# Matrixeigs/PowerSystemsReliabilityAssessment

Measured on AMD Instinct MI355X. Metric: Monte Carlo DC-OPF scenarios/sec (RTS-24 HL2 non-sequential), higher is better.
Workload: dtype f64

## Files before the change

powersystemsreliabilityassessment_amd/csrc/relmc_debug.hip:

```cpp
#include <cstdio>
#include <cstring>
#include <memory>

#include "relmc_ctx.h"
#include "relmc_shape_rts24.h"

using namespace relmc_host;

extern "C" {

int32_t relmc_debug_schedule(const relmc_ctx* ctx, int32_t* out9)
{
    if (!ctx || !out9 || !ctx->has_case) return RELMC_ERR_INVALID;
    auto fill = [&](const auto& C) {
        int ntask = 0;
        for (int p = 0; p < C.npass; ++p) ntask += C.pass_ntask[p];
        out9[0] = C.npass_upd; out9[1] = C.npass_inv; out9[2] = C.npass - C.npass_upd - C.npass_inv; out9[3] = C.noff;
        out9[4] = C.nzero; out9[5] = (int)C.nws; out9[6] = (int)ctx->lds_bytes; out9[7] = ctx->blocks_per_cu; out9[8] = ntask;
        if (verbose()) fprintf(stderr, "relmc: modelled LDS conflict cycles per Newton step %ld -> %ld\n", ctx->conflict_before, ctx->conflict_after);
        if (verbose()) fprintf(stderr, "relmc: longest line / injection list per bus slot: %d %d / %d %d\n", (int)C.maxdeg_s[0], (int)C.maxdeg_s[1], (int)C.maxinj_s[0], (int)C.maxinj_s[1]);
        if (verbose()) { fprintf(stderr, "relmc: tasks per pass:"); for (int p = 0; p < C.npass; ++p) fprintf(stderr, " %d", (int)C.pass_ntask[p]); fprintf(stderr, "\n"); }
    };
    if (ctx->tile == 0) fill(ctx->hcase24); else fill(ctx->hcase96);
    return RELMC_OK;
// ... 32 lines not shown
int32_t relmc_debug_phase_cycles(relmc_ctx* ctx, unsigned long long* out8)
{
    if (!ctx || !out8) return RELMC_ERR_INVALID;
    for (int k = 0; k < 8; ++k) out8[k] = 0;
    if (!ctx->dtiming.get() || ctx->timing_waves <= 0) return RELMC_OK;
    std::vector<unsigned long long> h((size_t)ctx->timing_waves * 8);
    HIP_TRY(ctx, hipMemcpy(h.data(), ctx->dtiming.get(), h.size() * sizeof(unsigned long long), hipMemcpyDeviceToHost));
    for (int w = 0; w < ctx->timing_waves; ++w) for (int k = 0; k < 8; ++k) out8[k] += h[(size_t)w * 8 + k];
    return RELMC_OK;
}

int32_t relmc_debug_norm_trips(relmc_ctx* ctx, unsigned long long* out2)
{
    if (!ctx || !out2) return RELMC_ERR_INVALID;
    out2[0] = out2[1] = 0;
    if (!ctx->dtiming.get() || ctx->timing_waves <= 0) return RELMC_OK;
    std::vector<unsigned long long> h((size_t)ctx->timing_waves * 2);
    HIP_TRY(ctx, hipMemcpy(h.data(), ctx->dtiming.get() + (size_t)ctx->timing_waves * 8, h.size() * sizeof(unsigned long long), hipMemcpyDeviceToHost));
    for (int w = 0; w < ctx->timing_waves; ++w) for (int k = 0; k < 2; ++k) out2[k] += h[(size_t)w * 2 + k];
    return RELMC_OK;
}

int32_t relmc_debug_trace(relmc_ctx* ctx, double* out, int32_t n_doubles)
{
    if (!ctx || !out || n_doubles < 0) return RELMC_ERR_INVALID;
    for (int k = 0; k < n_doubles; ++k) out[k] = 0.0;
    if (!ctx->dtiming.get() || n_doubles > 8 * 65536) return RELMC_OK;
    HIP_TRY(ctx, hipMemcpy(out, ctx->dtiming.get(), sizeof(double) * n_doubles, hipMemcpyDeviceToHost));
    return RELMC_OK;
}

int32_t relmc_debug_shape(const relmc_case_desc* d, const int32_t* order_hint, int32_t n_hint, int32_t* case_out, int32_t* static_out)
{
    if (static_out) ShapeRts24::values(static_out);
    if (case_out) {
        if (!d) return RELMC_ERR_INVALID;
        SymOpts so = sym_opts_default();
        if (order_hint && n_hint > 0) { so.order_hint = order_hint; so.n_hint = n_hint; }
        std::string err;
        SymGeom g;
        const int rc = with_symbolic(d, 0, so, g, err, [&](const auto& C) { shape_of(C, g.stash_off, g.scen_doubles, case_out); return (int)RELMC_OK; });
        if (rc) return rc < 0 ? rc : -rc;
    }
    return SF_COUNT;
}

int64_t relmc_debug_stretch_len(int64_t batch, int64_t done, double beta, double beta_limit, int64_t round, int32_t* final_out)
{
    if (batch <= 0 || batch > kStretchMaxBatch || done < 0 || round < 0) return RELMC_ERR_INVALID;
    const Stretch s = stretch_length(batch, done, beta, beta_limit, stretch_per(batch), round);
    if (final_out) *final_out = s.final ? 1 : 0;
    return s.len;
}

int32_t relmc_debug_shape_path(const relmc_ctx* ctx)
{
    if (!ctx || !ctx->has_case) return RELMC_ERR_INVALID;
    return ctx->shape_static && !ctx->sw.dynamic_shape ? 1 : 0;
}

int32_t relmc_debug_tail_plan(int64_t n, int32_t waves, int64_t* a_begin, int64_t* a_end, int32_t* owner, int64_t* group)
{
    if (n < 0 || waves <= 0) return RELMC_ERR_INVALID;
    const TailPlan plan(n, waves);
    for (int64_t w = 0; w < waves; ++w) { if (a_begin) a_begin[w] = plan.begin(w); if (a_end) a_end[w] = plan.cut(w); }
    for (int64_t p = 0; p < plan.items(); ++p) { if (owner) owner[p] = (int32_t)plan.owner(p); if (group) group[p] = plan.group(p); }
    return plan.T;
}

int32_t relmc_debug_tail_groups(const relmc_ctx* ctx, int64_t* launches_out, int32_t* waves_out)
{
    if (!ctx) return RELMC_ERR_INVALID;
    if (launches_out) *launches_out = ctx->tail_launches;
    if (waves_out) *waves_out = ctx->has_case && ctx->tile == 0 ? ctx->num_cu * ctx->blocks_per_cu * Tile24::WPB : 0;
    return ctx->last_tail_groups;
}

// ... 17 lines not shown
```

powersystemsreliabilityassessment_amd/csrc/relmc_dev.h:

```cpp
#pragma once
#include <stdint.h>

namespace relmc {

template <int RW_, int BS_, int LS_, int IS_, int NCOMPMAX_, int MAXPASS_, int MAXOFF_, int WPB_>
struct TileT {
    static constexpr int RW = RW_;
    static constexpr int BS = BS_;
    static constexpr int LS = LS_;
    static constexpr int IS = IS_;
    static constexpr int NBT = BS_ * RW_;
    static constexpr int NLT = LS_ * RW_;
    static constexpr int NIT = IS_ * RW_;
    static constexpr int SPW = 64 / RW_;
    static constexpr int NCOMPMAX = NCOMPMAX_;
    static constexpr int OW = NCOMPMAX_ / 32;
    static constexpr int MAXPASS = MAXPASS_;
    static constexpr int MAXOFF = MAXOFF_;
    static constexpr int WPB = WPB_;
    static_assert(BS_ <= 2 && LS_ <= 3 && IS_ <= 4, "the per-lane flag word has room for 2 bus, 3 line and 4 injection slots");
};
using Tile24 = TileT<16, 2, 3, 4, 128, 96, 160, 4>;
using Tile96 = TileT<64, 2, 2, 3, 256, 64, 320, 8>;
constexpr int DEGMAX = 8;
// ... 10 lines not shown
    static constexpr int NBT = TL::NBT, NLT = TL::NLT, NIT = TL::NIT, NCOMPMAX = TL::NCOMPMAX, MAXPASS = TL::MAXPASS, MAXOFF = TL::MAXOFF, ROWL = TL::RW;
    int32_t nb, ng, nl, nd, ninj, ncomp, ref_bus, noff;
    double base_mva, total_load;
    uint32_t exist_mask;
    uint32_t nws;
    uint16_t off_rhs, off_p;
    uint16_t npass, npass_upd, npass_inv, nzero;
    uint16_t maxdeg, maxinj, base_connected, npass_updq;
    uint16_t maxdeg_s[2], maxinj_s[2];
    uint16_t npass_updh, pad3[3];
    uint64_t bwd_half;
    uint64_t b_line8[NBT];
    uint64_t b_inj8[NBT];
    double b_bsum[NBT];
    double l_b[NLT];
    double l_rate[NLT];
    uint32_t l_info[NLT];
    int32_t l_partner[NLT];
    uint16_t l_blk[NLT];
    alignas(16) double i_tab[NIT][4];
    uint32_t i_info[NIT];
    uint8_t b_nline[NBT];
    uint8_t b_line[NBT][DEGMAX];
    uint8_t b_ninj[NBT];
    uint8_t b_inj[NBT][BINJMAX];
    int16_t b_vinj[NBT];
    uint8_t b_ext[NBT];
    uint8_t b_lane[NBT];
    uint8_t b_int[NBT];
    uint32_t thr[NCOMPMAX];
    uint16_t zero_off[MAXOFF];
    uint8_t pass_ntask[MAXPASS];
    uint16_t task[MAXPASS][ROWL][4];
};

template <class TL>
struct PartialT {
    double dns, dns2;
    double shed[TL::IS];
    uint32_t n, nfail, nsing, ninf, nnc, iters;
    uint32_t cf_inj[TL::IS];
    uint32_t cf_line[TL::LS];
    uint32_t pad;
};

template <class TL>
struct TailRecT {
    double shed[64][TL::IS];
    double dns[TL::SPW];
    uint32_t flag[TL::SPW];
};

struct FailRec {
    unsigned long long unit;
    uint32_t weight, pad;
    uint32_t mask[8];
};

struct EvalArgs {
    uint64_t seed, first_index;
    int64_t n;
    int32_t policy, max_it;
    double feastol, gradtol, comptol, costtol, xi, sigma, z0, alpha_min, max_stepsize;
    const uint8_t* states;
    double* dns;
    double* nodal;
// ... 139 lines not shown
```

powersystemsreliabilityassessment_amd/csrc/relmc_kernels.hip:

```cpp
#include "relmc_devfn.h"
#include "relmc_shape_rts24.h"

namespace relmc {


constexpr int kPrioBit = 12;
constexpr int kMinWaves = 2;
#define DINF __builtin_inf()
#define RELOAD_FENCE() __asm__ volatile("" ::: "memory")
#define SLOT_FENCE() __builtin_amdgcn_sched_barrier(0)
#ifdef RELMC_PASS_NOUNROLL
#define PASS_LOOP _Pragma("nounroll")
#else
#define PASS_LOOP
#endif
constexpr int kPfMask = 0xc0;
constexpr int kPfMaskWide = 0xc6;
#define PFSITE(k) (((PF_MASK >> (k)) & 1) != 0)
constexpr int kShadowMask = 0xff;
constexpr int kShadowMaskWide = 0xff;
constexpr int kNormSplitMask = 0xff;
constexpr int kNormSplitMaskWide = 0;
#ifdef RELMC_ZERO_EXPLICIT
constexpr bool kZeroBySlot = false;
#else
constexpr bool kZeroBySlot = true;
#endif
#define PASS_IDLE(d) (((d).x & 0xffffu) == ((d).y >> 16))
#define PASS_IDLE_INV(d) ((d).y != 0u)
#ifdef RELMC_PHASE_TIMING
#define PT_DECL unsigned long long pt_[8] = {0, 0, 0, 0, 0, 0, 0, 0}, ptn_[2] = {0, 0}; unsigned long long pt0_ = __builtin_readcyclecounter();
#define PT_MARK(k) { const unsigned long long n_ = __builtin_readcyclecounter(); pt_[k] += n_ - pt0_; pt0_ = n_; }
#define PT_TRIP(k) ptn_[k] += 1;
#define PT_FLUSH if (a.timing && lane == 0) { for (int k = 0; k < 8; ++k) a.timing[((size_t)blockIdx.x * WPB + (tid >> 6)) * 8 + k] = pt_[k]; \
                                              for (int k = 0; k < 2; ++k) a.timing[(size_t)gridDim.x * WPB * 8 + ((size_t)blockIdx.x * WPB + (tid >> 6)) * 2 + k] = ptn_[k]; }
#else
#define PT_DECL
#define PT_MARK(k)
#define PT_TRIP(k)
#define PT_FLUSH
#endif
#if defined(RELMC_PHASE_TIMING) && defined(RELMC_PT_INIT)
#undef PT_MARK
#define PT_MARK(k) { const unsigned long long n_ = __builtin_readcyclecounter(); pt_[(k) == 7 ? 7 : 6] += n_ - pt0_; pt0_ = n_; }
#define PT_IMARK(k) { const unsigned long long n_ = __builtin_readcyclecounter(); pt_[k] += n_ - pt0_; pt0_ = n_; }
#else
#define PT_IMARK(k)
#endif

template <int MODE_, class TL, class SH = ShapeDynamic>
__global__ void __launch_bounds__(64 * TL::WPB, kMinWaves) relmc_eval_kernel(const DevCaseT<TL>* __restrict__ gcase, const EvalArgs a)
{
    constexpr int MODE = MODE_ == 5 ? 0 : (MODE_ == 6 ? 4 : MODE_);
    constexpr bool DENSE = MODE_ == 6;
    constexpr int PAIR_MASK = TL::RW == 16 ? kRpairMask : kRpairMaskWide;
#define PAIRSITE(k) (((PAIR_MASK >> (k)) & 1) != 0)
    constexpr int PF_MASK = TL::RW == 16 ? kPfMask : kPfMaskWide;
    constexpr bool SHADOW = (((TL::RW == 16 ? kShadowMask : kShadowMaskWide) >> MODE) & 1) != 0;
    constexpr bool NSPLIT = (((TL::RW == 16 ? kNormSplitMask : kNormSplitMaskWide) >> MODE) & 1) != 0;
    constexpr bool LSHARE = (((TL::RW == 16 ? kLineRcpShareMask : kLineRcpShareMaskWide) >> MODE) & 1) != 0 && PAIRSITE(0) && PAIRSITE(2) && PAIRSITE(6);
    constexpr bool ZSLOT = kZeroBySlot && (SH::kMask & SH::grp_nl) != 0 && (SH::kMask & SH::grp_ninj) != 0;
    constexpr int RW = TL::RW, BS = TL::BS, LS = TL::LS, IS = TL::IS, NBT = TL::NBT, WPB = TL::WPB, SPW = TL::SPW, OW = TL::OW;
    using DevCase = DevCaseT<TL>;
    using Partial = PartialT<TL>;
    extern __shared__ __attribute__((aligned(16))) unsigned char smem[];
    constexpr uint32_t OPT_BYTES = 128;
    double* const OPT = reinterpret_cast<double*>(smem);
#define A_(k, name) OPT[k]
    DevCase& C = *reinterpret_cast<DevCase*>(smem + OPT_BYTES);
    const DevCase& TASKSRC = *gcase;
    const DevCase& TABL = C;
    const DevCase& TABI = (RW == 64) ? *gcase : C;
    const DevCase& TABG = (RW == 64) ? *gcase : C;
    const int tid = threadIdx.x, lane = tid & 63, rlane = lane & (RW - 1), row = tid / RW;
    const uint32_t case_bytes = a.case_bytes;
    {
        const uint32_t* src = reinterpret_cast<const uint32_t*>(gcase);
        uint32_t* dst = reinterpret_cast<uint32_t*>(smem + OPT_BYTES);
        if (tid == 0) { OPT[0] = a.feastol; OPT[1] = a.gradtol; OPT[2] = a.comptol; OPT[3] = a.costtol; OPT[4] = a.xi; OPT[5] = a.sigma;
                        OPT[6] = a.z0; OPT[7] = a.alpha_min; OPT[8] = a.max_stepsize; OPT[9] = a.fail_threshold; }
        for (uint32_t i = tid; i < case_bytes / 4; i += 64 * WPB) dst[i] = src[i];
    }
    __syncthreads();
    double* const W = reinterpret_cast<double*>(smem + OPT_BYTES + ((case_bytes + 15u) & ~15u)) + (size_t)row * SHAPE(scen_doubles, a.scen_doubles);
    const int nlp = SHAPE(nl, C.nl), nip = SHAPE(ninj, C.ninj);
    double* const LR = W;
    double* const IR = W + 4 * (nlp + 1);
    const int maxdeg0 = SHAPE(maxdeg0, C.maxdeg_s[0]), maxdeg1 = SHAPE(maxdeg1, C.maxdeg_s[1]), maxinj0 = SHAPE(maxinj0, C.maxinj_s[0]), maxinj1 = SHAPE(maxinj1, C.maxinj_s[1]);
    double* const Stash = W + SHAPE(stash_off, a.stash_off) + 2 * rlane;
    const double* const StashJ = W + SHAPE(stash_off, a.stash_off);
    double* const Lam = W + SHAPE(stash_off, a.stash_off) + 2 * IS * RW + 2;
    uint32_t* const OB = reinterpret_cast<uint32_t*>(Lam + NBT);

    const int ng = SHAPE(ng, C.ng), ncomp = C.ncomp, nb = SHAPE(nb, C.nb);
    const bool bwd_all_half = SHAPE(bwd_all_half, __builtin_amdgcn_readfirstlane((uint32_t)(C.bwd_half != 0 ? 1u : 0u)) != 0);
    const int off_rhs = SHAPE(off_rhs, C.off_rhs), npu = SHAPE(npass_upd, C.npass_upd), npi = SHAPE(npass_inv, C.npass_inv), npass = SHAPE(npass, C.npass), nzero = SHAPE(nzero, C.nzero), npuh = SHAPE(npass_upd, C.npass_upd) - SHAPE(npass_updq, C.npass_updq), npuf = npuh - SHAPE(npass_updh, C.npass_updh);
    const double base = C.base_mva;
    const double eps = 2.220446049250313e-16;

    uint32_t linfo[LS]; int lpart[LS];
#pragma unroll
    for (int s = 0; s < LS; ++s) { const int l = RW * s + rlane; linfo[s] = C.l_info[l]; lpart[s] = C.l_partner[l]; }
    constexpr bool LTAB_LDS = (MODE == 1 || MODE == 2 || MODE == 4);
    constexpr bool ITAB_REG = RW == 64;
    double lbv_[LS], lrv_[LS], ihi_[IS], ilo_[IS];
#pragma unroll
    for (int s = 0; s < LS; ++s) { lbv_[s] = LTAB_LDS ? 0.0 : TABL.l_b[RW * s + rlane]; lrv_[s] = LTAB_LDS ? 0.0 : TABL.l_rate[RW * s + rlane]; }
#pragma unroll
    for (int s = 0; s < IS; ++s) { ihi_[s] = ITAB_REG ? TABI.i_tab[RW * s + rlane][0] : 0.0; ilo_[s] = ITAB_REG ? TABI.i_tab[RW * s + rlane][1] : 0.0; }
#define lb(s) (LTAB_LDS ? TABL.l_b[RW * (s) + rlane] : lbv_[s])
#define lr(s) (LTAB_LDS ? TABL.l_rate[RW * (s) + rlane] : lrv_[s])
#define IHL(s, j) (ITAB_REG ? d2{ihi_[s], ilo_[s]} : ld2(TABI.i_tab[j]))
#define ICOST(s, j) TABI.i_tab[j][2]
#define PLIST(t, bi) TABG.b_line8[bi]
#define JLIST(t, bi) TABG.b_inj8[bi]
    uint32_t iinfo[IS];
#pragma unroll
    for (int s = 0; s < IS; ++s) iinfo[s] = C.i_info[RW * s + rlane];
    int vb[BS];
#pragma unroll
    for (int t = 0; t < BS; ++t) vb[t] = C.b_lane[RW * t + rlane];

    Partial& PA = reinterpret_cast<Partial*>(a.partial)[(size_t)blockIdx.x * (64 * WPB) + tid];
    {
        PA.dns = 0.0; PA.dns2 = 0.0;
#pragma unroll
        for (int s = 0; s < IS; ++s) { PA.shed[s] = 0.0; PA.cf_inj[s] = 0; }
#pragma unroll
        for (int s = 0; s < LS; ++s) PA.cf_line[s] = 0;
        PA.n = 0; PA.nfail = 0; PA.nsing = 0; PA.ninf = 0; PA.nnc = 0; PA.iters = 0; PA.pad = 0;
    }
    uint32_t acc_n = 0, acc_it = 0;

    PT_DECL
    const int64_t ngroups = (a.n + SPW - 1) / SPW;
    const int64_t gwave = (int64_t)blockIdx.x * WPB + (tid >> 6);
    const int64_t gstride = (int64_t)gridDim.x * WPB;
    const bool prio_first = a.prio_mode == 1 ? blockIdx.x < (gridDim.x >> 1) : (a.prio_mode == 2 ? ((tid >> 8) & 1) == 0 : false);
    if (a.prio_mode != 0 && !prio_first) __builtin_amdgcn_s_setprio(1);
    constexpr bool WINDOWED = (MODE == 0 && RW == 16);
    uint32_t* const WIN = reinterpret_cast<uint32_t*>(smem + OPT_BYTES + ((case_bytes + 15u) & ~15u)) +
                          (size_t)SPW * WPB * SHAPE(scen_doubles, a.scen_doubles) * 2 + (size_t)(tid >> 6) * 256;
    uint8_t* const WINL = reinterpret_cast<uint8_t*>(smem + OPT_BYTES + ((case_bytes + 15u) & ~15u)) +
                          ((size_t)SPW * WPB * SHAPE(scen_doubles, a.scen_doubles) * 2 + (size_t)WPB * 256) * 4 + (size_t)(tid >> 6) * 64;
    int64_t wb_begin = gwave, wb_end = ngroups, wb_step = gstride;
    if (WINDOWED) {
        wb_begin = ngroups * gwave / gstride; wb_end = ngroups * (gwave + 1) / gstride; wb_step = 16;
    }
    static_assert(!WINDOWED || 80 + 4 * WPB <= OPT_BYTES, "one word per wavefront behind the ten option doubles");
    int* const TP = reinterpret_cast<int*>(smem + 80) + (tid >> 6);
    if (WINDOWED) { *TP = -1; RELOAD_FENCE(); }
    for (int64_t wb = wb_begin; WINDOWED || wb < wb_end; wb += wb_step) {
    int win_groups = 1, wg0 = 0;
    uint32_t win_valid = 0;
// ... 510 lines not shown
                        const double hp = pv - hl.x, hm = ILOV(s, hl.y) - pv;
                        const double lxp = ICOST(s, j) - Lam[iinfo[s] & 0xff] + (imup[s] - imum[s]);
                        if constexpr ((RW == 16 && kInjNform) || (RW == 64 && kInjNformWide)) {
                            const double N = __builtin_fma(imup[s], izm[s], imum[s] * izp[s]);
                            const double rN = frcp(N), zz = izp[s] * izm[s];
                            invD = zz * rN;
                            npd = __builtin_fma(lxp, zz, (imup[s] * hp + gamma) * izm[s] - (imum[s] * hm + gamma) * izp[s]) * rN;
                        } else {
                        double rzp, rzm; frcp_pair<PAIRSITE(1)>(izp[s], izm[s], rzp, rzm);
                        const double D = imup[s] * rzp + imum[s] * rzm;
                        const double np = lxp + (imup[s] * hp + gamma) * rzp - (imum[s] * hm + gamma) * rzm;
                        invD = frcp(D); npd = np * invD;
                        }
                        if constexpr (NORMS) {
                            mx_lx = vmax(mx_lx, __builtin_fabs(lxp));
                            mx_gh = vmax(mx_gh, vmax(hp, hm));
                            mx_z = vmax(mx_z, vmax(izp[s], izm[s]));
                            mx_lammu = vmax(mx_lammu, vmax(imup[s], imum[s]));
                        }
                    }
                    if (ZSLOT ? j <= nip : j < nip) IR[j] = pv;
                    st2(Stash + 2 * RW * s, invD, npd);
                    SLOT_FENCE();
                }
                PT_MARK(1)
                if (rlane == 0) {
                    if (!ZSLOT || nlp >= LS * RW) { st2(LR + 4 * nlp, 0.0, 0.0); st2(LR + 4 * nlp + 2, 0.0, 0.0); }
                    if (!ZSLOT || nip >= IS * RW) IR[nip] = 0.0;
                }
                uint32_t lblk_pf[LS]; uint32_t zo_pf = 0;
                if constexpr (PFSITE(1)) {
#pragma unroll
                    for (int s = 0; s < LS; ++s) lblk_pf[s] = C.l_blk[RW * s + rlane];
                    zo_pf = C.zero_off[rlane];
                }
                unsigned long long pl_pf[BS], pj_pf[BS];
                if constexpr (PFSITE(2)) {
#pragma unroll
                    for (int t = 0; t < BS; ++t) { const int bq = vb[t] < nb ? vb[t] : 0; pl_pf[t] = PLIST(t, bq); pj_pf[t] = JLIST(t, bq); }
                }
                double vown[LS];
                {
                    double gp[LS];
#pragma unroll
                    for (int s = 0; s < LS; ++s) gp[s] = LR[4 * (lpart[s] >= 0 ? lpart[s] : nlp)];
#pragma unroll
                    for (int s = 0; s < LS; ++s) vown[s] = (((linfo[s] >> 24) & LF_OWNER) && !L_PIN(s)) ? -(gown[s] + gp[s]) : 0.0;
                }
                double d00[BS], d11[BS], r0[BS], r1[BS];
#pragma unroll
                for (int t = 0; t < BS; ++t) {
                    const int bi = vb[t];
                    d00[t] = 0; d11[t] = 0; r0[t] = 0; r1[t] = 0;
                    if (bi < nb) {
                        double md = 0.0, lx = 0.0, nq_ = 0.0, bal = 0.0, E = 0.0, ssum = 0.0;
                        const unsigned long long pl = PFSITE(2) ? pl_pf[t] : PLIST(t, bi), pj = PFSITE(2) ? pj_pf[t] : JLIST(t, bi);
#pragma unroll
                        for (int e = 0; e < DEGMAX; e += 2) {
                            if (e >= (t == 0 ? maxdeg0 : maxdeg1)) break;
                            const uint32_t ent0 = (uint32_t)(pl >> (8 * e)) & 0xffu, ent1 = (uint32_t)(pl >> (8 * e + 8)) & 0xffu;
                            const int l0 = (int)(ent0 & 0x7f), l1 = (int)(ent1 & 0x7f);
                            const double sg0 = (ent0 & 0x80) ? -1.0 : 1.0, sg1 = (ent1 & 0x80) ? -1.0 : 1.0;
                            const d2 ra0 = ld2(LR + 4 * l0), rb0 = ld2(LR + 4 * l0 + 2), ra1 = ld2(LR + 4 * l1), rb1 = ld2(LR + 4 * l1 + 2);
                            md += ra0.x;
                            lx = __builtin_fma(sg0, ra0.y, lx);
                            nq_ = __builtin_fma(sg0, rb0.x, nq_);
                            bal = __builtin_fma(sg0, rb0.y, bal);
// ... 32 lines not shown
                }
                double o_ct = 0.0, o_cc = 0.0, o_am = 0.0;
                if constexpr (NSPLIT && PFSITE(7)) o_am = A_(7, alpha_min);
                RELOAD_FENCE();
                if constexpr (DENSE) {
                    const int n = 2 * nb, n1 = n + 1;
                    volatile double* A = a.dense + ((size_t)blockIdx.x * (WPB * SPW) + (size_t)(tid / RW)) * (size_t)a.dense_stride;
                    for (int e = rlane; e < n * n1; e += RW) A[e] = 0.0;
                    __threadfence_block();
#pragma unroll
                    for (int s = 0; s < LS; ++s) {
                        if ((linfo[s] >> 24) & LF_OWNER) {
                            const int f = linfo[s] & 0xff, t = (linfo[s] >> 8) & 0xff;
                            const int hi = f < t ? t : f, lo = f < t ? f : t;
                            const double c1 = L_C1Z(s) ? 0.0 : cBv[s], c2 = L_C2Z(s) ? 0.0 : cBv[s];
                            A[(2 * hi) * n1 + 2 * lo] = vown[s]; A[(2 * lo) * n1 + 2 * hi] = vown[s];
                            A[(2 * hi) * n1 + 2 * lo + 1] = c1; A[(2 * lo + 1) * n1 + 2 * hi] = c1;
                            A[(2 * hi + 1) * n1 + 2 * lo] = c2; A[(2 * lo) * n1 + 2 * hi + 1] = c2;
                        }
                    }
#pragma unroll
                    for (int t = 0; t < BS; ++t) {
                        const int bi = vb[t];
                        if (bi < nb) {
                            A[(2 * bi) * n1 + 2 * bi] = d00[t]; A[(2 * bi) * n1 + 2 * bi + 1] = cBd[t];
                            A[(2 * bi + 1) * n1 + 2 * bi] = cBd[t]; A[(2 * bi + 1) * n1 + 2 * bi + 1] = d11[t];
                            A[(2 * bi) * n1 + n] = r0[t]; A[(2 * bi + 1) * n1 + n] = r1[t];
                        }
                    }
                    __threadfence_block();
                } else {
#pragma unroll
                for (int s = 0; s < LS; ++s) {
                    if ((linfo[s] >> 24) & LF_OWNER) {
                        const double c1 = L_C1Z(s) ? 0.0 : cBv[s];
                        const double c2 = L_C2Z(s) ? 0.0 : cBv[s];
                        double* blk = W + (PFSITE(1) ? lblk_pf[s] : (uint32_t)C.l_blk[RW * s + rlane]);
                        st2(blk, vown[s], c1); st2(blk + 2, c2, 0.0);
                    }
                }
                if constexpr (PFSITE(1)) {
                    for (int z = rlane; z < nzero; z += RW) {
                        const uint32_t zn = C.zero_off[z + RW < TL::MAXOFF ? z + RW : z];
                        double* blk = W + zo_pf; st2(blk, 0.0, 0.0); st2(blk + 2, 0.0, 0.0);
                        zo_pf = zn;
                    }
                } else
                for (int z = rlane; z < nzero; z += RW) { double* blk = W + C.zero_off[z]; st2(blk, 0.0, 0.0); st2(blk + 2, 0.0, 0.0); }
#pragma unroll
                for (int t = 0; t < BS; ++t) {
                    const int bi = vb[t];
                    if (bi < nb) {
                        st2(W + 4 * bi, d00[t], cBd[t]); st2(W + 4 * bi + 2, cBd[t], d11[t]);
                        st2(W + off_rhs + 2 * bi, r0[t], r1[t]);
                    }
                }
                }

                PT_MARK(2)
                bool conv = false, xnan = false;
                if constexpr (NSPLIT) {
                    mx_x = x_inf; xnan = x_nan;
                    conv = NORMS && stage1;
                } else {
                    if constexpr (PFSITE(7)) { o_ct = A_(2, comptol); o_cc = A_(3, costtol); o_am = A_(7, alpha_min); }
                    mx_x = row_max<RW>(mx_x);
                    xnan = row_any<RW>(nanx, lane);
                    if constexpr (!PFSITE(7)) { o_ct = A_(2, comptol); o_cc = A_(3, costtol); }
                    conv = it > 0 && zmu < o_ct * (1.0 + mx_x) && __builtin_fabs(fval - f0) < o_cc * (1.0 + __builtin_fabs(f0));
                }
#ifdef RELMC_TRACE
                {
                    const double t_gh = row_max<RW>(mx_gh), t_z = row_max<RW>(mx_z), t_lx = row_max<RW>(mx_lx), t_lm = row_max<RW>(mx_lammu);
                    if (a.timing && blockIdx.x == 0 && tid == 0 && it < 60) {
                        double* o = reinterpret_cast<double*>(a.timing) + 8 * it;
                        o[0] = t_gh / (1.0 + vmax(mx_x, t_z)); o[1] = t_lx / (1.0 + t_lm); o[2] = zmu / (1.0 + mx_x);
                        o[3] = __builtin_fabs(fval - f0) / (1.0 + __builtin_fabs(f0)); o[4] = alphap; o[5] = alphad; o[6] = gamma; o[7] = fval;
                    }
                }
#endif
                if constexpr (NORMS) if (__any(conv)) {
                    mx_gh = row_max<RW>(mx_gh); mx_z = row_max<RW>(mx_z); mx_lx = row_max<RW>(mx_lx); mx_lammu = row_max<RW>(mx_lammu);
                    conv = conv && mx_gh < A_(0, feastol) * (1.0 + vmax(mx_x, mx_z)) && mx_lx < A_(1, gradtol) * (1.0 + mx_lammu);
                }
// ... 559 lines not shown
```

powersystemsreliabilityassessment_amd/csrc/relmc_schedule.hip:

```cpp
#include <algorithm>
#include <chrono>
#include <cmath>
#include <cstddef>
#include <cstdio>
#include <cstdlib>
#include <cstring>

#include "relmc_ctx.h"
#ifdef RELMC_DEV_SWITCHES
#include "relmc_dev_switches.h"
#endif

namespace relmc_host {

bool verbose()
{
    static const bool v = std::getenv("RELMC_VERBOSE") != nullptr;
    return v;
}

SymOpts sym_opts_default()
{
    SymOpts so;
#ifdef RELMC_DEV_SWITCHES
// ... 562 lines not shown
        }
        C.maxdeg = (uint16_t)maxdeg; C.maxinj = (uint16_t)maxinj;
        return RELMC_OK;
    }
    void bus_lanes()
    {
        for (int q = 0; q < NBT; ++q) C.b_lane[q] = 0xff;
        std::vector<int> slot_of(nb, 0);
        const int n1 = nb > ROWL ? nb - ROWL : 0;
        if (n1 > 0 && TL::BS == 2 && !so.no_bus_map) {
            int best_a = DEGMAX, best_b = BINJMAX, best_steps = 1 << 30;
            for (int a2 = 0; a2 <= DEGMAX; ++a2) for (int b2 = 0; b2 <= BINJMAX; ++b2) {
                int cnt = 0;
                for (int i = 0; i < nb; ++i) if (C.b_nline[i] <= a2 && C.b_ninj[i] <= b2) cnt++;
                const int steps = (a2 + 1) / 2 + (b2 + 1) / 2;
                if (cnt >= n1 && steps < best_steps) { best_steps = steps; best_a = a2; best_b = b2; }
            }
            std::vector<int> cand;
            for (int i = 0; i < nb; ++i) if (C.b_nline[i] <= best_a && C.b_ninj[i] <= best_b) cand.push_back(i);
            std::stable_sort(cand.begin(), cand.end(), [&](int x, int y) { return C.b_nline[x] + C.b_ninj[x] < C.b_nline[y] + C.b_ninj[y]; });
            for (int k = 0; k < n1; ++k) slot_of[cand[k]] = 1;
        } else {
            for (int i = 0; i < nb; ++i) slot_of[i] = i / ROWL;
        }
        int fill[TL::BS] = {};
        for (int i = 0; i < nb; ++i) {
            const int t = slot_of[i];
            C.b_lane[ROWL * t + fill[t]++] = (uint8_t)i;
            if (C.b_nline[i] > C.maxdeg_s[t]) C.maxdeg_s[t] = C.b_nline[i];
            if (C.b_ninj[i] > C.maxinj_s[t]) C.maxinj_s[t] = C.b_ninj[i];
        }
    }

    void base_connectivity()
    {
        std::vector<int> lab(nb); for (int i = 0; i < nb; ++i) lab[i] = i;
        auto find = [&](int x) { while (lab[x] != x) { lab[x] = lab[lab[x]]; x = lab[x]; } return x; };
        for (int l = 0; l < nl; ++l) { const int a2 = find(d->br_from[l]), b2 = find(d->br_to[l]); if (a2 != b2) lab[a2] = b2; }
        int roots = 0; for (int i = 0; i < nb; ++i) if (find(i) == i) roots++;
        C.base_connected = roots == 1 ? 1 : 0;
    }

    void thresholds()
    {
        for (int k = 0; k < ncomp; ++k) {
            double t = std::floor(d->unavail[k] * 4294967296.0);
            if (!(t > 0)) t = 0;
            if (t > 4294967295.0) t = 4294967295.0;
            C.thr[k] = d->always_up[k] ? 0u : (uint32_t)t;
        }
    }
    int geometry()
    {
        const uint32_t case_bytes = (uint32_t)offsetof(DevCaseT<TL>, task);
        const uint32_t lds_bytes = 128u + ((case_bytes + 15u) & ~15u) + (uint32_t)SPW * WPB * stride * (uint32_t)sizeof(double) + (ROWL == 16 ? (1024u + 64u) * WPB : 0u);
        if (lds_bytes > 160u * 1024u) return failx(RELMC_ERR_UNSUPPORTED, "relmc_case_load: case needs more than 160 KiB of LDS per workgroup");
        geom.stash_off = stash_off; geom.scen_doubles = stride; geom.lds_bytes = lds_bytes;
        return RELMC_OK;
    }
};

}

template <class TL>
int case_symbolic(const relmc_case_desc* d, DevCaseT<TL>& C, int order_variant, const SymOpts& so, SymGeom& geom, std::string& err)
{
    using S = Symbolic<TL>;
    using clock = std::chrono::steady_clock;
    auto ms = [](clock::time_point a, clock::time_point b) { return std::chrono::duration<double, std::milli>(b - a).count(); };
    S s(d, C, order_variant, so, geom, err);
    auto run = [&](std::initializer_list<int (S::*)()> steps) { for (auto step : steps) if (const int rc = (s.*step)()) return rc; return (int)RELMC_OK; };
    if (const int rc = run({&S::header, &S::elimination_order, &S::block_layout, &S::task_list})) return rc;
    const auto t_sched0 = clock::now();
    s.dependencies();
    if (const int rc = s.schedule()) return rc;
    const auto t_place0 = clock::now();
    if (verbose()) fprintf(stderr, "relmc: scheduling %.1f ms\n", ms(t_sched0, t_place0));
    s.place();
    if (verbose()) fprintf(stderr, "relmc: placement search %.1f ms\n", ms(t_place0, clock::now()));
    s.pass_forms();
    s.byte_offsets();
    if (const int rc = run({&S::shadow_idle_lanes, &S::pass_counts, &S::lines, &S::injections})) return rc;
    s.bus_lanes();
    s.base_connectivity();
    s.thresholds();
    return s.geometry();
}

template int case_symbolic<Tile24>(const relmc_case_desc*, DevCaseT<Tile24>&, int, const SymOpts&, SymGeom&, std::string&);
template int case_symbolic<Tile96>(const relmc_case_desc*, DevCaseT<Tile96>&, int, const SymOpts&, SymGeom&, std::string&);

constexpr long kPassWeight = 4;
template <class TL>
long schedule_cost(const DevCaseT<TL>& C, int32_t* lds_out, int32_t* passes_out)
{
    const int nbwd = (int)C.npass - (int)C.npass_upd - (int)C.npass_inv;
    const int nfull = (int)C.npass_upd - (int)C.npass_updh - (int)C.npass_updq;
    long lds = 10L * nfull + 7L * C.npass_updh + 6L * C.npass_updq + 6L * C.npass_inv;
    for (int k = 0; k < nbwd; ++k) lds += (k < 64 && ((C.bwd_half >> k) & 1ull)) ? 6 : 7;
    if (lds_out) *lds_out = (int32_t)lds;
    if (passes_out) *passes_out = (int32_t)C.npass;
    return lds + kPassWeight * (long)C.npass;
}
template <class TL>
int tune_order_impl(const relmc_case_desc* d, DevCaseT<TL>& C, int32_t evaluations, uint64_t seed, const int32_t* start, int32_t* order_out, int32_t* stats)
{
    const int nb = d->nb;
    SymOpts so = sym_opts_default();
    so.place_moves = 0;
    std::string err;
    SymGeom g;
    std::vector<int32_t> cur(nb), best(nb), cand(nb);
    int32_t lds = 0, np = 0;
    if (start) cur.assign(start, start + nb);
    else {
        const int rc = case_symbolic<TL>(d, C, 0, so, g, err);
// ... 105 lines not shown
```

powersystemsreliabilityassessment_amd/csrc/relmc_shape.h:

```cpp
#pragma once
#include <stdint.h>

#include "relmc_dev.h"

namespace relmc {

enum ShapeField {
    SF_RW = 0, SF_NB, SF_NG, SF_NL, SF_NINJ, SF_NZERO, SF_OFF_RHS, SF_NPASS_UPD, SF_NPASS_UPDH, SF_NPASS_UPDQ, SF_NPASS_INV, SF_NPASS,
    SF_MAXDEG0, SF_MAXDEG1, SF_MAXINJ0, SF_MAXINJ1, SF_BWD_ALL_HALF, SF_STASH_OFF, SF_SCEN_DOUBLES, SF_COUNT
};

enum ShapeGroup { SG_PASS = 1, SG_GATHER = 2, SG_DIM = 4, SG_OFF = 8, SG_ALL = 15 };
#define SHAPE(field, dyn) ((SH::kMask & SH::grp_##field) != 0 ? (decltype(+(dyn)))SH::field : (dyn))
struct ShapeGroups {
    static constexpr int grp_npass_upd = SG_PASS, grp_npass_updh = SG_PASS, grp_npass_updq = SG_PASS, grp_npass_inv = SG_PASS, grp_npass = SG_PASS, grp_bwd_all_half = SG_PASS,
                         grp_maxdeg0 = SG_GATHER, grp_maxdeg1 = SG_GATHER, grp_maxinj0 = SG_GATHER, grp_maxinj1 = SG_GATHER,
                         grp_nb = SG_DIM, grp_ng = SG_DIM, grp_nl = SG_DIM, grp_ninj = SG_DIM, grp_nzero = SG_DIM,
                         grp_off_rhs = SG_OFF, grp_stash_off = SG_OFF, grp_scen_doubles = SG_OFF;
};
struct ShapeDynamic : ShapeGroups {
    static constexpr int kMask = 0;
    static constexpr int nb = 0, ng = 0, nl = 0, ninj = 0, nzero = 0, off_rhs = 0, npass_upd = 0, npass_updh = 0, npass_updq = 0, npass_inv = 0, npass = 0,
                         maxdeg0 = 0, maxdeg1 = 0, maxinj0 = 0, maxinj1 = 0, bwd_all_half = 0, stash_off = 0, scen_doubles = 0;
};

template <class V, int MASK = SG_ALL>
struct ShapeStaticT : ShapeGroups {
    static constexpr int kMask = MASK;
    static constexpr int nb = V::nb, ng = V::ng, nl = V::nl, ninj = V::ninj, nzero = V::nzero, off_rhs = V::off_rhs, npass_upd = V::npass_upd, npass_updh = V::npass_updh,
                         npass_updq = V::npass_updq, npass_inv = V::npass_inv, npass = V::npass, maxdeg0 = V::maxdeg0, maxdeg1 = V::maxdeg1, maxinj0 = V::maxinj0,
                         maxinj1 = V::maxinj1, bwd_all_half = V::bwd_all_half, stash_off = V::stash_off, scen_doubles = V::scen_doubles;
    static void values(int32_t* out)
    {
        out[SF_RW] = V::rw; out[SF_NB] = V::nb; out[SF_NG] = V::ng; out[SF_NL] = V::nl; out[SF_NINJ] = V::ninj; out[SF_NZERO] = V::nzero;
        out[SF_OFF_RHS] = V::off_rhs; out[SF_NPASS_UPD] = V::npass_upd; out[SF_NPASS_UPDH] = V::npass_updh; out[SF_NPASS_UPDQ] = V::npass_updq;
        out[SF_NPASS_INV] = V::npass_inv; out[SF_NPASS] = V::npass; out[SF_MAXDEG0] = V::maxdeg0; out[SF_MAXDEG1] = V::maxdeg1;
        out[SF_MAXINJ0] = V::maxinj0; out[SF_MAXINJ1] = V::maxinj1; out[SF_BWD_ALL_HALF] = V::bwd_all_half; out[SF_STASH_OFF] = V::stash_off;
        out[SF_SCEN_DOUBLES] = V::scen_doubles;
    }
};

template <class DC>
inline void shape_of(const DC& C, uint32_t stash_off, uint32_t scen_doubles, int32_t* out)
{
    out[SF_RW] = DC::ROWL; out[SF_NB] = C.nb; out[SF_NG] = C.ng; out[SF_NL] = C.nl; out[SF_NINJ] = C.ninj; out[SF_NZERO] = C.nzero;
    out[SF_OFF_RHS] = C.off_rhs; out[SF_NPASS_UPD] = C.npass_upd; out[SF_NPASS_UPDH] = C.npass_updh; out[SF_NPASS_UPDQ] = C.npass_updq;
    out[SF_NPASS_INV] = C.npass_inv; out[SF_NPASS] = C.npass; out[SF_MAXDEG0] = C.maxdeg_s[0]; out[SF_MAXDEG1] = C.maxdeg_s[1];
    out[SF_MAXINJ0] = C.maxinj_s[0]; out[SF_MAXINJ1] = C.maxinj_s[1]; out[SF_BWD_ALL_HALF] = C.bwd_half != 0 ? 1 : 0; out[SF_STASH_OFF] = (int32_t)stash_off;
    out[SF_SCEN_DOUBLES] = (int32_t)scen_doubles;
}

template <class SH, class DC>
inline bool shape_matches(const DC& C, uint32_t stash_off, uint32_t scen_doubles)
{
    int32_t a[SF_COUNT], b[SF_COUNT];
    SH::values(a); shape_of(C, stash_off, scen_doubles, b);
    for (int k = 0; k < SF_COUNT; ++k) if (a[k] != b[k]) return false;
    return true;
}

}
```

powersystemsreliabilityassessment_amd/csrc/relmc_shape_rts24.h:

```cpp
#pragma once
#include "relmc_shape.h"

namespace relmc {

struct ShapeRts24Values {
    static constexpr int rw = 16;
    static constexpr int nb = 24;
    static constexpr int ng = 33;
    static constexpr int nl = 38;
    static constexpr int ninj = 50;
    static constexpr int nzero = 20;
    static constexpr int off_rhs = 312;
    static constexpr int npass_upd = 12;
    static constexpr int npass_updh = 3;
    static constexpr int npass_updq = 1;
    static constexpr int npass_inv = 2;
    static constexpr int npass = 21;
    static constexpr int maxdeg0 = 5;
    static constexpr int maxdeg1 = 3;
    static constexpr int maxinj0 = 7;
    static constexpr int maxinj1 = 1;
    static constexpr int bwd_all_half = 0;
    static constexpr int stash_off = 360;
    static constexpr int scen_doubles = 526;
};
#ifndef RELMC_SHAPE_MASK
#define RELMC_SHAPE_MASK (SG_PASS | SG_DIM | SG_OFF)
#endif
using ShapeRts24 = ShapeStaticT<ShapeRts24Values, RELMC_SHAPE_MASK>;

}
```

Before: 64.28 million.

## Clear fill blocks with idle line and bus lanes instead of a separate zero loop

Fill-in blocks that were zeroed by a separate strided loop each Newton step are assigned at load time to idle line-slot and bus-slot lanes. Those lanes now store zero blocks as part of their normal assembly stores. A host-side swap search places the fill offsets to reduce modelled LDS bank conflicts, and the shared-memory case copy substitutes the fill-augmented line block table. For RTS-24 the residual zero loop becomes empty, at the cost of more case metadata, extra shape fields and a global-memory read of the bus lane table.

New measurement: 66.03 million, median of 6. 1.03x the previous value.

```diff
diff --git a/powersystemsreliabilityassessment_amd/csrc/relmc_debug.hip b/powersystemsreliabilityassessment_amd/csrc/relmc_debug.hip
--- a/powersystemsreliabilityassessment_amd/csrc/relmc_debug.hip
+++ b/powersystemsreliabilityassessment_amd/csrc/relmc_debug.hip
@@ -88,17 +88,40 @@
 
 int32_t relmc_debug_shape(const relmc_case_desc* d, const int32_t* order_hint, int32_t n_hint, int32_t* case_out, int32_t* static_out)
 {
-    if (static_out) ShapeRts24::values(static_out);
+    int32_t v[SF_COUNT_ALL];
+    if (static_out) { ShapeRts24::values(v); std::memcpy(static_out, v, sizeof(int32_t) * SF_COUNT); }
     if (case_out) {
         if (!d) return RELMC_ERR_INVALID;
         SymOpts so = sym_opts_default();
         if (order_hint && n_hint > 0) { so.order_hint = order_hint; so.n_hint = n_hint; }
         std::string err;
         SymGeom g;
-        const int rc = with_symbolic(d, 0, so, g, err, [&](const auto& C) { shape_of(C, g.stash_off, g.scen_doubles, case_out); return (int)RELMC_OK; });
+        const int rc = with_symbolic(d, 0, so, g, err, [&](const auto& C) { shape_of(C, g.stash_off, g.scen_doubles, v); return (int)RELMC_OK; });
         if (rc) return rc < 0 ? rc : -rc;
+        std::memcpy(case_out, v, sizeof(int32_t) * SF_COUNT);
     }
     return SF_COUNT;
+}
+
+int32_t relmc_debug_fill_lanes(const relmc_case_desc* d, int32_t order_variant, const int32_t* order_hint, int32_t n_hint, int32_t* hdr, uint16_t* l_blk_fill,
+                               uint16_t* b_lane_fill, uint8_t* b_lane)
+{
+    if (!d || !hdr) return RELMC_ERR_INVALID;
+    SymOpts so = sym_opts_default();
+    if (order_hint && n_hint > 0) { so.order_hint = order_hint; so.n_hint = n_hint; }
+    std::string err;
+    SymGeom g;
+    return with_symbolic(d, order_variant, so, g, err, [&](const auto& C) {
+        using DC = std::decay_t<decltype(C)>;
+        int32_t st[SF_COUNT_ALL];
+        ShapeRts24::values(st);
+        hdr[0] = DC::ROWL; hdr[1] = C.nb; hdr[2] = C.nl; hdr[3] = C.nzero; hdr[4] = C.nzero_res; hdr[5] = C.nfill_line; hdr[6] = C.nfill_bus; hdr[7] = DC::NLT; hdr[8] = DC::NBT;
+        hdr[9] = st[SF_NZERO_RES]; hdr[10] = st[SF_NFILL_BUS];
+        hdr[11] = C.nidle_line; hdr[12] = C.nidle_bus_s[0]; hdr[13] = C.nidle_bus_s[1]; hdr[14] = st[SF_NIDLE_LINE]; hdr[15] = st[SF_NIDLE_BUS0]; hdr[16] = st[SF_NIDLE_BUS1];
+        for (int l = 0; l < DC::NLT; ++l) if (l_blk_fill) l_blk_fill[l] = C.l_blk_fill[l];
+        for (int q = 0; q < DC::NBT; ++q) { if (b_lane_fill) b_lane_fill[q] = C.b_lane_fill[q]; if (b_lane) b_lane[q] = C.b_lane[q]; }
+        return (int)RELMC_OK;
+    });
 }
 
 int64_t relmc_debug_stretch_len(int64_t batch, int64_t done, double beta, double beta_limit, int64_t round, int32_t* final_out)
diff --git a/powersystemsreliabilityassessment_amd/csrc/relmc_dev.h b/powersystemsreliabilityassessment_amd/csrc/relmc_dev.h
--- a/powersystemsreliabilityassessment_amd/csrc/relmc_dev.h
+++ b/powersystemsreliabilityassessment_amd/csrc/relmc_dev.h
@@ -66,6 +66,11 @@
     uint16_t zero_off[MAXOFF];
     uint8_t pass_ntask[MAXPASS];
     uint16_t task[MAXPASS][ROWL][4];
+    uint16_t l_blk_fill[NLT];
+    uint16_t b_lane_fill[NBT];
+    uint16_t nzero_res, nfill_line, nfill_bus;
+    uint16_t nidle_line, nidle_bus_s[2];
+    uint16_t pad4[2];
 };
 
 template <class TL>
diff --git a/powersystemsreliabilityassessment_amd/csrc/relmc_kernels.hip b/powersystemsreliabilityassessment_amd/csrc/relmc_kernels.hip
--- a/powersystemsreliabilityassessment_amd/csrc/relmc_kernels.hip
+++ b/powersystemsreliabilityassessment_amd/csrc/relmc_kernels.hip
@@ -26,6 +26,11 @@
 #else
 constexpr bool kZeroBySlot = true;
 #endif
+#ifdef RELMC_FILL_LOOP
+constexpr bool kFillBySlot = false;
+#else
+constexpr bool kFillBySlot = true;
+#endif
 #define PASS_IDLE(d) (((d).x & 0xffffu) == ((d).y >> 16))
 #define PASS_IDLE_INV(d) ((d).y != 0u)
 #ifdef RELMC_PHASE_TIMING
@@ -60,6 +65,8 @@
     constexpr bool NSPLIT = (((TL::RW == 16 ? kNormSplitMask : kNormSplitMaskWide) >> MODE) & 1) != 0;
     constexpr bool LSHARE = (((TL::RW == 16 ? kLineRcpShareMask : kLineRcpShareMaskWide) >> MODE) & 1) != 0 && PAIRSITE(0) && PAIRSITE(2) && PAIRSITE(6);
     constexpr bool ZSLOT = kZeroBySlot && (SH::kMask & SH::grp_nl) != 0 && (SH::kMask & SH::grp_ninj) != 0;
+    constexpr bool FSLOT = kFillBySlot && !DENSE && (SH::kMask & SH::grp_nzero_res) != 0 && (SH::kMask & SH::grp_nfill_bus) != 0;
+    constexpr bool FBUS = FSLOT && SH::nfill_bus > 0;
     constexpr int RW = TL::RW, BS = TL::BS, LS = TL::LS, IS = TL::IS, NBT = TL::NBT, WPB = TL::WPB, SPW = TL::SPW, OW = TL::OW;
     using DevCase = DevCaseT<TL>;
     using Partial = PartialT<TL>;
@@ -79,6 +86,11 @@
         uint32_t* dst = reinterpret_cast<uint32_t*>(smem + OPT_BYTES);
         if (tid == 0) { OPT[0] = a.feastol; OPT[1] = a.gradtol; OPT[2] = a.comptol; OPT[3] = a.costtol; OPT[4] = a.xi; OPT[5] = a.sigma;
                         OPT[6] = a.z0; OPT[7] = a.alpha_min; OPT[8] = a.max_stepsize; OPT[9] = a.fail_threshold; }
+        if constexpr (FSLOT) {
+            constexpr uint32_t LB0 = offsetof(DevCase, l_blk) / 4, LBN = sizeof(DevCase::l_blk) / 4, LF0 = offsetof(DevCase, l_blk_fill) / 4;
+            static_assert(offsetof(DevCase, l_blk) % 4 == 0 && sizeof(DevCase::l_blk) % 4 == 0 && offsetof(DevCase, l_blk_fill) % 4 == 0, "l_blk and l_blk_fill are copied as 32-bit words");
+            for (uint32_t i = tid; i < case_bytes / 4; i += 64 * WPB) dst[i] = src[i - LB0 < LBN ? LF0 + (i - LB0) : i];
+        } else
         for (uint32_t i = tid; i < case_bytes / 4; i += 64 * WPB) dst[i] = src[i];
     }
     __syncthreads();
@@ -119,7 +131,7 @@
     for (int s = 0; s < IS; ++s) iinfo[s] = C.i_info[RW * s + rlane];
     int vb[BS];
 #pragma unroll
-    for (int t = 0; t < BS; ++t) vb[t] = C.b_lane[RW * t + rlane];
+    for (int t = 0; t < BS; ++t) vb[t] = FBUS ? (int)gcase->b_lane_fill[RW * t + rlane] : (int)C.b_lane[RW * t + rlane];
 
     Partial& PA = reinterpret_cast<Partial*>(a.partial)[(size_t)blockIdx.x * (64 * WPB) + tid];
     {
@@ -696,7 +708,7 @@
                 if constexpr (PFSITE(1)) {
 #pragma unroll
                     for (int s = 0; s < LS; ++s) lblk_pf[s] = C.l_blk[RW * s + rlane];
-                    zo_pf = C.zero_off[rlane];
+                    if constexpr (!FSLOT) zo_pf = C.zero_off[rlane];
                 }
                 unsigned long long pl_pf[BS], pj_pf[BS];
                 if constexpr (PFSITE(2)) {
@@ -795,24 +807,32 @@
                 } else {
 #pragma unroll
                 for (int s = 0; s < LS; ++s) {
-                    if ((linfo[s] >> 24) & LF_OWNER) {
+                    const uint32_t lbf = FSLOT ? (PFSITE(1) ? lblk_pf[s] : (uint32_t)C.l_blk[RW * s + rlane]) : 0u;
+                    if (FSLOT ? (SHAPE(nidle_line, 1) == 0 || lbf != 0xffffu) : ((linfo[s] >> 24) & LF_OWNER) != 0) {
                         const double c1 = L_C1Z(s) ? 0.0 : cBv[s];
                         const double c2 = L_C2Z(s) ? 0.0 : cBv[s];
-                        double* blk = W + (PFSITE(1) ? lblk_pf[s] : (uint32_t)C.l_blk[RW * s + rlane]);
+                        double* blk = W + (FSLOT ? lbf : (PFSITE(1) ? lblk_pf[s] : (uint32_t)C.l_blk[RW * s + rlane]));
                         st2(blk, vown[s], c1); st2(blk + 2, c2, 0.0);
                     }
                 }
-                if constexpr (PFSITE(1)) {
+                const int nzloop = FSLOT ? SHAPE(nzero_res, 0) : nzero;
+                if constexpr (PFSITE(1) && !FSLOT) {
                     for (int z = rlane; z < nzero; z += RW) {
                         const uint32_t zn = C.zero_off[z + RW < TL::MAXOFF ? z + RW : z];
                         double* blk = W + zo_pf; st2(blk, 0.0, 0.0); st2(blk + 2, 0.0, 0.0);
                         zo_pf = zn;
                     }
                 } else
-                for (int z = rlane; z < nzero; z += RW) { double* blk = W + C.zero_off[z]; st2(blk, 0.0, 0.0); st2(blk + 2, 0.0, 0.0); }
+                for (int z = rlane; z < nzloop; z += RW) { double* blk = W + C.zero_off[z]; st2(blk, 0.0, 0.0); st2(blk + 2, 0.0, 0.0); }
 #pragma unroll
                 for (int t = 0; t < BS; ++t) {
                     const int bi = vb[t];
+                    if constexpr (FBUS) {
+                        if ((t == 0 ? SHAPE(nidle_bus0, 1) : SHAPE(nidle_bus1, 1)) == 0 || bi != 0xffff) {
+                            st2(W + 4 * bi, d00[t], cBd[t]); st2(W + 4 * bi + 2, cBd[t], d11[t]);
+                            if (bi < nb) st2(W + off_rhs + 2 * bi, r0[t], r1[t]);
+                        }
+                    } else
                     if (bi < nb) {
                         st2(W + 4 * bi, d00[t], cBd[t]); st2(W + 4 * bi + 2, cBd[t], d11[t]);
                         st2(W + off_rhs + 2 * bi, r0[t], r1[t]);
diff --git a/powersystemsreliabilityassessment_amd/csrc/relmc_schedule.hip b/powersystemsreliabilityassessment_amd/csrc/relmc_schedule.hip
--- a/powersystemsreliabilityassessment_amd/csrc/relmc_schedule.hip
+++ b/powersystemsreliabilityassessment_amd/csrc/relmc_schedule.hip
@@ -618,6 +618,64 @@
         }
     }
 
+    long fill_slot_cost(const uint16_t* off) const
+    {
+        long cyc = 0;
+        for (int g = 0; g < ROWL / 8; ++g) {
+            int n[8] = {}, mx = 0; uint16_t seen[8][8];
+            for (int r = 8 * g; r < 8 * g + 8; ++r) {
+                if (off[r] == 0xffff) continue;
+                const int set = (off[r] / 2) & 7;
+                bool dup = false; for (int k = 0; k < n[set]; ++k) dup = dup || seen[set][k] == off[r];
+                if (!dup) seen[set][n[set]++] = off[r];
+                if (n[set] > mx) mx = n[set];
+            }
+            cyc += mx;
+        }
+        cyc *= SPW;
+        return 2 * (cyc > 13 ? cyc : 13);
+    }
+    int fill_lanes()
+    {
+        for (int l = 0; l < NLT; ++l) C.l_blk_fill[l] = ((C.l_info[l] >> 24) & LF_OWNER) ? C.l_blk[l] : (uint16_t)0xffff;
+        std::vector<uint16_t> boff(NBT);
+        for (int q = 0; q < NBT; ++q) boff[q] = C.b_lane[q] == 0xff ? (uint16_t)0xffff : (uint16_t)(4 * C.b_lane[q]);
+        std::vector<uint16_t*> spare;
+        for (int l = 0; l < NLT; ++l) if (C.l_blk_fill[l] == 0xffff) spare.push_back(&C.l_blk_fill[l]);
+        const int nspare_line = (int)spare.size();
+        for (int q = 0; q < NBT; ++q) if (boff[q] == 0xffff) spare.push_back(&boff[q]);
+        const int nres = C.nzero > spare.size() ? C.nzero - (int)spare.size() : 0;
+        for (int z = nres; z < C.nzero; ++z) if (C.zero_off[z] < 4 * nb || C.zero_off[z] % 4) return failx(RELMC_ERR_INVALID, "relmc_case_load: fill block among the diagonal blocks");
+        auto slot_of = [&](const uint16_t* t) { return t >= boff.data() && t < boff.data() + NBT ? boff.data() + (t - boff.data()) / ROWL * ROWL : C.l_blk_fill + (t - C.l_blk_fill) / ROWL * ROWL; };
+        for (int z = nres, k = 0; z < C.nzero; ++z, ++k) *spare[k] = C.zero_off[z];
+        for (int sweep = 0; sweep < 8 && so.place_moves > 0; ++sweep) {
+            bool better = false;
+            for (size_t i = 0; i < spare.size(); ++i) for (size_t j = i + 1; j < spare.size(); ++j) {
+                if (*spare[i] == *spare[j]) continue;
+                const uint16_t* si = slot_of(spare[i]); const uint16_t* sj = slot_of(spare[j]);
+                const long before = fill_slot_cost(si) + (sj != si ? fill_slot_cost(sj) : 0);
+                std::swap(*spare[i], *spare[j]);
+                const long after = fill_slot_cost(si) + (sj != si ? fill_slot_cost(sj) : 0);
+                if (after < before) better = true; else std::swap(*spare[i], *spare[j]);
+            }
+            if (!better) break;
+        }
+        int nline = 0, nbus = 0;
+        for (int k = 0; k < (int)spare.size(); ++k) if (*spare[k] != 0xffff) { if (k < nspare_line) nline++; else nbus++; }
+        for (int q = 0; q < NBT; ++q) C.b_lane_fill[q] = boff[q] == 0xffff ? (uint16_t)0xffff : (uint16_t)(boff[q] / 4);
+        C.nfill_line = (uint16_t)nline; C.nfill_bus = (uint16_t)nbus; C.nzero_res = (uint16_t)nres;
+        C.nidle_line = 0; C.nidle_bus_s[0] = C.nidle_bus_s[1] = 0;
+        for (int l = 0; l < NLT; ++l) if (C.l_blk_fill[l] == 0xffff) C.nidle_line++;
+        for (int q = 0; q < NBT; ++q) if (C.b_lane_fill[q] == 0xffff) C.nidle_bus_s[q / ROWL]++;
+        if (verbose()) {
+            long cyc = 0;
+            for (int t = 0; t < NLT / ROWL; ++t) cyc += fill_slot_cost(C.l_blk_fill + ROWL * t);
+            for (int t = 0; t < NBT / ROWL; ++t) cyc += fill_slot_cost(boff.data() + ROWL * t);
+            fprintf(stderr, "relmc: order %d: %d fill blocks: %d cleared by line-slot lanes, %d by bus-slot lanes, %d by the loop; modelled LDS cycles of the block stores %ld\n", order_variant, (int)C.nzero, nline, nbus, nres, cyc);
+        }
+        return RELMC_OK;
+    }
+
     void base_connectivity()
     {
         std::vector<int> lab(nb); for (int i = 0; i < nb; ++i) lab[i] = i;
@@ -668,6 +726,7 @@
     s.byte_offsets();
     if (const int rc = run({&S::shadow_idle_lanes, &S::pass_counts, &S::lines, &S::injections})) return rc;
     s.bus_lanes();
+    if (const int rc = s.fill_lanes()) return rc;
     s.base_connectivity();
     s.thresholds();
     return s.geometry();
diff --git a/powersystemsreliabilityassessment_amd/csrc/relmc_shape.h b/powersystemsreliabilityassessment_amd/csrc/relmc_shape.h
--- a/powersystemsreliabilityassessment_amd/csrc/relmc_shape.h
+++ b/powersystemsreliabilityassessment_amd/csrc/relmc_shape.h
@@ -7,7 +7,8 @@
 
 enum ShapeField {
     SF_RW = 0, SF_NB, SF_NG, SF_NL, SF_NINJ, SF_NZERO, SF_OFF_RHS, SF_NPASS_UPD, SF_NPASS_UPDH, SF_NPASS_UPDQ, SF_NPASS_INV, SF_NPASS,
-    SF_MAXDEG0, SF_MAXDEG1, SF_MAXINJ0, SF_MAXINJ1, SF_BWD_ALL_HALF, SF_STASH_OFF, SF_SCEN_DOUBLES, SF_COUNT
+    SF_MAXDEG0, SF_MAXDEG1, SF_MAXINJ0, SF_MAXINJ1, SF_BWD_ALL_HALF, SF_STASH_OFF, SF_SCEN_DOUBLES, SF_COUNT,
+    SF_NZERO_RES = SF_COUNT, SF_NFILL_BUS, SF_NIDLE_LINE, SF_NIDLE_BUS0, SF_NIDLE_BUS1, SF_COUNT_ALL
 };
 
 enum ShapeGroup { SG_PASS = 1, SG_GATHER = 2, SG_DIM = 4, SG_OFF = 8, SG_ALL = 15 };
@@ -15,19 +16,19 @@
 struct ShapeGroups {
     static constexpr int grp_npass_upd = SG_PASS, grp_npass_updh = SG_PASS, grp_npass_updq = SG_PASS, grp_npass_inv = SG_PASS, grp_npass = SG_PASS, grp_bwd_all_half = SG_PASS,
                          grp_maxdeg0 = SG_GATHER, grp_maxdeg1 = SG_GATHER, grp_maxinj0 = SG_GATHER, grp_maxinj1 = SG_GATHER,
-                         grp_nb = SG_DIM, grp_ng = SG_DIM, grp_nl = SG_DIM, grp_ninj = SG_DIM, grp_nzero = SG_DIM,
+                         grp_nb = SG_DIM, grp_ng = SG_DIM, grp_nl = SG_DIM, grp_ninj = SG_DIM, grp_nzero = SG_DIM, grp_nzero_res = SG_DIM, grp_nfill_bus = SG_DIM, grp_nidle_line = SG_DIM, grp_nidle_bus0 = SG_DIM, grp_nidle_bus1 = SG_DIM,
                          grp_off_rhs = SG_OFF, grp_stash_off = SG_OFF, grp_scen_doubles = SG_OFF;
 };
 struct ShapeDynamic : ShapeGroups {
     static constexpr int kMask = 0;
-    static constexpr int nb = 0, ng = 0, nl = 0, ninj = 0, nzero = 0, off_rhs = 0, npass_upd = 0, npass_updh = 0, npass_updq = 0, npass_inv = 0, npass = 0,
+    static constexpr int nb = 0, ng = 0, nl = 0, ninj = 0, nzero = 0, nzero_res = 0, nfill_bus = 0, nidle_line = 0, nidle_bus0 = 0, nidle_bus1 = 0, off_rhs = 0, npass_upd = 0, npass_updh = 0, npass_updq = 0, npass_inv = 0, npass = 0,
                          maxdeg0 = 0, maxdeg1 = 0, maxinj0 = 0, maxinj1 = 0, bwd_all_half = 0, stash_off = 0, scen_doubles = 0;
 };
 
 template <class V, int MASK = SG_ALL>
 struct ShapeStaticT : ShapeGroups {
     static constexpr int kMask = MASK;
-    static constexpr int nb = V::nb, ng = V::ng, nl = V::nl, ninj = V::ninj, nzero = V::nzero, off_rhs = V::off_rhs, npass_upd = V::npass_upd, npass_updh = V::npass_updh,
+    static constexpr int nb = V::nb, ng = V::ng, nl = V::nl, ninj = V::ninj, nzero = V::nzero, nzero_res = V::nzero_res, nfill_bus = V::nfill_bus, nidle_line = V::nidle_line, nidle_bus0 = V::nidle_bus0, nidle_bus1 = V::nidle_bus1, off_rhs = V::off_rhs, npass_upd = V::npass_upd, npass_updh = V::npass_updh,
                          npass_updq = V::npass_updq, npass_inv = V::npass_inv, npass = V::npass, maxdeg0 = V::maxdeg0, maxdeg1 = V::maxdeg1, maxinj0 = V::maxinj0,
                          maxinj1 = V::maxinj1, bwd_all_half = V::bwd_all_half, stash_off = V::stash_off, scen_doubles = V::scen_doubles;
     static void values(int32_t* out)
@@ -36,7 +37,8 @@
         out[SF_OFF_RHS] = V::off_rhs; out[SF_NPASS_UPD] = V::npass_upd; out[SF_NPASS_UPDH] = V::npass_updh; out[SF_NPASS_UPDQ] = V::npass_updq;
         out[SF_NPASS_INV] = V::npass_inv; out[SF_NPASS] = V::npass; out[SF_MAXDEG0] = V::maxdeg0; out[SF_MAXDEG1] = V::maxdeg1;
         out[SF_MAXINJ0] = V::maxinj0; out[SF_MAXINJ1] = V::maxinj1; out[SF_BWD_ALL_HALF] = V::bwd_all_half; out[SF_STASH_OFF] = V::stash_off;
-        out[SF_SCEN_DOUBLES] = V::scen_doubles;
+        out[SF_SCEN_DOUBLES] = V::scen_doubles; out[SF_NZERO_RES] = V::nzero_res; out[SF_NFILL_BUS] = V::nfill_bus;
+        out[SF_NIDLE_LINE] = V::nidle_line; out[SF_NIDLE_BUS0] = V::nidle_bus0; out[SF_NIDLE_BUS1] = V::nidle_bus1;
     }
 };
 
@@ -47,15 +49,16 @@
     out[SF_OFF_RHS] = C.off_rhs; out[SF_NPASS_UPD] = C.npass_upd; out[SF_NPASS_UPDH] = C.npass_updh; out[SF_NPASS_UPDQ] = C.npass_updq;
     out[SF_NPASS_INV] = C.npass_inv; out[SF_NPASS] = C.npass; out[SF_MAXDEG0] = C.maxdeg_s[0]; out[SF_MAXDEG1] = C.maxdeg_s[1];
     out[SF_MAXINJ0] = C.maxinj_s[0]; out[SF_MAXINJ1] = C.maxinj_s[1]; out[SF_BWD_ALL_HALF] = C.bwd_half != 0 ? 1 : 0; out[SF_STASH_OFF] = (int32_t)stash_off;
-    out[SF_SCEN_DOUBLES] = (int32_t)scen_doubles;
+    out[SF_SCEN_DOUBLES] = (int32_t)scen_doubles; out[SF_NZERO_RES] = C.nzero_res; out[SF_NFILL_BUS] = C.nfill_bus;
+    out[SF_NIDLE_LINE] = C.nidle_line; out[SF_NIDLE_BUS0] = C.nidle_bus_s[0]; out[SF_NIDLE_BUS1] = C.nidle_bus_s[1];
 }
 
 template <class SH, class DC>
 inline bool shape_matches(const DC& C, uint32_t stash_off, uint32_t scen_doubles)
 {
-    int32_t a[SF_COUNT], b[SF_COUNT];
+    int32_t a[SF_COUNT_ALL], b[SF_COUNT_ALL];
     SH::values(a); shape_of(C, stash_off, scen_doubles, b);
-    for (int k = 0; k < SF_COUNT; ++k) if (a[k] != b[k]) return false;
+    for (int k = 0; k < SF_COUNT_ALL; ++k) if (a[k] != b[k]) return false;
     return true;
 }
 
diff --git a/powersystemsreliabilityassessment_amd/csrc/relmc_shape_rts24.h b/powersystemsreliabilityassessment_amd/csrc/relmc_shape_rts24.h
--- a/powersystemsreliabilityassessment_amd/csrc/relmc_shape_rts24.h
+++ b/powersystemsreliabilityassessment_amd/csrc/relmc_shape_rts24.h
@@ -23,6 +23,11 @@
     static constexpr int bwd_all_half = 0;
     static constexpr int stash_off = 360;
     static constexpr int scen_doubles = 526;
+    static constexpr int nzero_res = 0;
+    static constexpr int nfill_bus = 6;
+    static constexpr int nidle_line = 0;
+    static constexpr int nidle_bus0 = 0;
+    static constexpr int nidle_bus1 = 2;
 };
 #ifndef RELMC_SHAPE_MASK
 #define RELMC_SHAPE_MASK (SG_PASS | SG_DIM | SG_OFF)
```
